# protolambda/go-kzg

Measured on AMD Instinct MI355X. Metric: KZG commitments/sec (CommitToPoly, 4096-element blob); FK20 half: value_fk20_4096, higher is better.
Workload: dtype u32; 1 GPU; CommitToPoly, 4096-coeff blobs, eth/trusted_setup.json monomial setup (s=1337), 4096 blobs/step/GPU resident in HBM, fixed-base table budget 110 GB (library default 110 GB: signed 16-bit windows, 8 of them walked by both GLV halves of every scalar, 103 GB; see table_sweep); global_batch=4096, parallelism=dp1 (independent blobs, no data-path collective)

## Files before the change

go-kzg_amd/csrc/capi_fk20.hip:

```cpp
#include "capi_common.hpp"

__global__ void k_fk20_x(const g1j *secret, uint64_t n, uint64_t l, uint64_t k, g1j *x ) {
    uint64_t t = blockIdx.x * (uint64_t)blockDim.x + threadIdx.x;
    if (t >= l * k) return;
    uint64_t off = t / k, i = t % k;
    x[t] = (i + 1 < k) ? secret[n - l - 1 - off - i * l] : g1_inf();
}

static int fk20_core_new(kzg_hip_kzg *ks, uint64_t n2, uint64_t l, fk20_core *c) {
    kzg_hip_fft *fs = ks->fs;
    dev_guard g(fs);
    hipStream_t s = fs->stream;
    uint64_t n = n2 / 2, k = n / l, k2 = 2 * k;
    c->ks = ks; c->n2 = n2; c->l = l; c->k = k;
    dtmp<g1j> d_x(s), d_f(s);
    CHK(d_x.alloc(l * k)); CHK(d_f.alloc(l * k2));
    HIPCHK(hipMalloc((void **)&c->d_files, l * k2 * sizeof(g1j)));
    hipLaunchKernelGGL(k_fk20_x, dim3((uint32_t)((l * k + 255) / 256)), dim3(256), 0, s, ks->d_secret, n, l, k, d_x.p);
    CHK(g1_fft_rows(fs, s, d_x.p, k, k, d_f.p, k2, l, 0));
    launch_g1_normalize(s, d_f.p, c->d_files, l * k2);
    HIPCHK(hipGetLastError());
    {
        double budget_gb = table_budget_gb("KZG_HIP_FK20_FB_BUDGET_GB", 48.0, 12.0);
        uint64_t npts = l * k2;
        const bool glv = fb_glv_enabled();
        dtmp<g1a> d_fa(s);
        if (npts >= 64) { CHK(d_fa.alloc(npts)); launch_g1_to_affine(s, c->d_files, d_fa.p, npts); }
        for (uint32_t cc = glv ? 16 : 14; cc >= 4 && npts >= 64; cc--) {
            const uint32_t nwin = glv ? fb_windows_glv(cc) : fb_windows(cc);
            if (glv && cc > 4 && fb_windows_glv(cc - 1) == nwin) continue;
            double bytes = (double)nwin * (double)npts * (double)(1u << (cc - 1)) * sizeof(g1a);
            if (bytes > budget_gb * 1e9) continue;
            g1a *tab = nullptr;
            if (hipMalloc((void **)&tab, (size_t)nwin * npts * (1u << (cc - 1)) * sizeof(g1a)) != hipSuccess) { (void)hipGetLastError(); continue; }
            hipError_t e = launch_fb_build(s, d_fa.p, npts, cc, nwin, tab);
            if (e == hipSuccess) e = hipStreamSynchronize(s);
            if (e != hipSuccess) { (void)hipGetLastError(); hipFree(tab); continue; }
            c->d_files_fb = tab; c->fb_c = cc; c->fb_nwin = nwin; c->fb_glv = glv;
            break;
        }
    }
    HIPCHK(hipStreamSynchronize(s));
    return KZG_HIP_OK;
}

int fk20_hext(fk20_core *c, hipStream_t s, const fr *d_poly, uint64_t poly_stride, uint64_t n, uint64_t batch, uint64_t j0, uint64_t cnt, g1j *d_hext) {
    kzg_hip_fft *fs = c->ks->fs;
    uint64_t l = c->l, k2 = 2 * c->k;
    dtmp<fr> d_tc(s), d_cf(s);
    CHK(d_tc.alloc(batch * l * k2)); CHK(d_cf.alloc(batch * l * k2));
    launch_toeplitz_coeffs(s, d_poly, poly_stride, n, l, batch, d_tc.p, fs->d_inv_pow2 + ilog2(k2));
    fr_fft_rows(fs, s, d_tc.p, k2, k2, d_cf.p, k2, batch * l, 0);
    if (c->d_files_fb) {
        if (l == 1) launch_fb_mul_vec(s, c->d_files_fb, l * k2, c->fb_c, c->fb_nwin, d_cf.p, k2, j0, cnt, batch, d_hext, c->fb_glv);
        else if (batch * cnt >= device_simd_lanes()) launch_fb_mul_vec_files(s, c->d_files_fb, l * k2, c->fb_c, c->fb_nwin, d_cf.p, k2, j0, cnt, batch, d_hext, c->fb_glv);
        else {
            dtmp<g1j> d_tmp(s);
            CHK(d_tmp.alloc(batch * l * cnt));
            launch_fb_mul_vec(s, c->d_files_fb, l * k2, c->fb_c, c->fb_nwin, d_cf.p, k2, j0, cnt, batch, d_tmp.p, c->fb_glv);
            launch_g1_sum_files(s, d_tmp.p, l, cnt, batch, d_hext);
        }
// ... 13 lines not shown
    HIPCHK(hipGetLastError());
    return KZG_HIP_OK;
}
int fk20_finish(fk20_core *c, hipStream_t s, const g1j *d_hext, uint64_t batch, int da, int bit_reverse, g1j *d_out) {
    kzg_hip_fft *fs = c->ks->fs;
    const uint64_t k2 = 2 * c->k;
    dtmp<g1j> d_a(s);
    CHK(d_a.alloc(batch * k2));
    CHK(g1_fft_rows(fs, s, d_hext, k2, k2, d_a.p, k2, batch, 1, nullptr, c->k));
    return fk20_finish_from_h(c, s, d_a.p, batch, da, bit_reverse, d_out);
}
static bool fk20_pass1_fused_ok(const fk20_core *c, uint64_t batch) {
    static const bool off = [] { const char *e = getenv("KZG_HIP_FK20_PASS1"); return e && e[0] == '0'; }();
    const uint64_t k2 = 2 * c->k;
    return !off && c->l == 1 && c->d_files_fb && k2 >= 32 && g1_fft_direct_mode(k2, batch) && g1_fft_direct_logr(k2, batch) == 4;
}
static int fk20_run_pass1_fused(fk20_core *c, hipStream_t s, const fr *d_poly, uint64_t poly_stride, uint64_t n, uint64_t batch, int da, int bit_reverse, g1j *d_out) {
    kzg_hip_fft *fs = c->ks->fs;
    const uint64_t k2 = 2 * c->k;
    dtmp<fr> d_tc(s), d_cf(s); dtmp<g1j> d_p1(s), d_a(s), d_tmp(s);
    CHK(d_tc.alloc(batch * k2)); CHK(d_cf.alloc(batch * k2)); CHK(d_p1.alloc(batch * k2)); CHK(d_a.alloc(batch * k2)); CHK(d_tmp.alloc(batch * k2));
    launch_toeplitz_coeffs(s, d_poly, poly_stride, n, 1, batch, d_tc.p, fs->d_inv_pow2 + ilog2(k2));
    fr_fft_rows(fs, s, d_tc.p, k2, k2, d_cf.p, k2, batch, 0);
    launch_fb_direct_pass1(s, c->d_files_fb, k2, c->fb_c, c->fb_nwin, d_cf.p, fs->d_reversed, fs->W, batch, 4, d_p1.p, c->fb_glv);
    launch_g1_fft_direct(s, d_p1.p, k2, k2, d_a.p, d_tmp.p, k2, batch, fs->d_reversed, fs->W, nullptr, 4, g1_fft_direct_lanes(k2, batch), 4, c->k);
    HIPCHK(hipGetLastError());
    return fk20_finish_from_h(c, s, d_a.p, batch, da, bit_reverse, d_out);
}
static bool fk20_fused_ok(const fk20_core *c, uint64_t batch, int da) {
    static const bool off = [] { const char *e = getenv("KZG_HIP_FK20_FUSE"); return e && e[0] == '0'; }();
    const uint64_t k2 = 2 * c->k;
    return !off && c->l == 1 && c->d_files_fb && k2 >= 8 && !g1_fft_direct_mode(k2, batch) && (da || !g1_fft_direct_mode(c->k, batch));
}
static int fk20_run_fused(fk20_core *c, hipStream_t s, const fr *d_poly, uint64_t poly_stride, uint64_t n, uint64_t batch, int da, int bit_reverse, g1j *d_out) {
    kzg_hip_fft *fs = c->ks->fs;
    const uint64_t k2 = 2 * c->k;
    dtmp<fr> d_tc(s), d_cf(s); dtmp<g1j> d_a(s), d_b(s);
    CHK(d_tc.alloc(batch * k2)); CHK(d_cf.alloc(batch * k2)); CHK(d_a.alloc(batch * k2)); CHK(d_b.alloc(batch * k2));
    launch_toeplitz_coeffs(s, d_poly, poly_stride, n, 1, batch, d_tc.p, fs->d_inv_pow2 + ilog2(k2));
    fr_fft_rows(fs, s, d_tc.p, k2, k2, d_cf.p, k2, batch, 0);
    launch_fb_mul_vec_dif2(s, c->d_files_fb, k2, c->fb_c, c->fb_nwin, d_cf.p, fs->d_reversed, fs->W, batch, d_a.p, c->fb_glv);
    for (uint64_t m = k2 / 8; m >= 1; m >>= 1) launch_g1_fft_stage_dif(s, d_a.p, k2, batch, m, fs->d_glv_reversed, fs->d_wnaf_reversed, fs->W);
    if (!da) {
        const uint64_t k = c->k;
        launch_g1_take_even(s, d_a.p, d_b.p, batch * k);
        for (uint64_t m = 1; m < k; m <<= 1) launch_g1_fft_stage(s, d_b.p, k, batch, m, fs->d_glv_expanded, fs->d_wnaf_expanded, fs->W);
        if (bit_reverse) { launch_g1_bitrev_copy(s, d_b.p, k, k, d_a.p, k, batch); launch_g1_normalize(s, d_a.p, d_out, batch * k, true); }
        else launch_g1_normalize(s, d_b.p, d_out, batch * k, true);
        HIPCHK(hipGetLastError());
        return KZG_HIP_OK;
    }
    launch_g1_clear_odd(s, d_a.p, batch * k2);
    for (uint64_t m = 1; m < k2; m <<= 1) launch_g1_fft_stage(s, d_a.p, k2, batch, m, fs->d_glv_expanded, fs->d_wnaf_expanded, fs->W);
    if (bit_reverse) { launch_g1_bitrev_copy(s, d_a.p, k2, k2, d_b.p, k2, batch); launch_g1_normalize(s, d_b.p, d_out, batch * k2, true); }
    else launch_g1_normalize(s, d_a.p, d_out, batch * k2, true);
    HIPCHK(hipGetLastError());
    return KZG_HIP_OK;
}
static uint64_t fk20_padded_batch(uint64_t batch) {
    static const bool off = [] { const char *e = getenv("KZG_HIP_FK20_PAD"); return e && e[0] == '0'; }();
    if (off) return batch;
    if (batch > 16 && batch < 32) return 32;
    if (batch > 32 && (batch & 7)) {
        const uint64_t p = (batch + 7) & ~7ull;
        if ((p - batch) * 32 <= batch) return p;
    }
    return batch;
// ... 222 lines not shown
```

go-kzg_amd/csrc/g1_coop_kernels.hpp:

```cpp
#pragma once
#include "internal.hpp"
#include "g1_quad.hpp"
#include <stdlib.h>
#include <string.h>

namespace kzg {

#ifndef G1_BLOCK
#define G1_BLOCK 256
#endif
struct g1jq_slot { uint32_t w[39]; uint32_t inf; uint32_t pad; };
#define G1_DIRECT_BLOCK 64
static inline uint32_t ilog2_coop(uint64_t v) { uint32_t r = 0; while ((1ull << r) < v) r++; return r; }

template <bool DIF, bool WNAF, int L> __global__ __launch_bounds__(G1_BLOCK, 2) void k_g1_fft_stage_quad(g1j *data, uint32_t logn, uint64_t m, const fr *roots, const int8_t *wnaf, uint64_t W, uint64_t total, uint64_t batch) {
    const uint64_t t4 = blockIdx.x * (uint64_t)blockDim.x + threadIdx.x;
    const uint32_t role = (uint32_t)(t4 & (uint64_t)(L - 1));
    const uint64_t t = t4 / L;
    if (t >= total) return;
    const uint64_t half = 1ull << (logn - 1), groups = half / m;
    const uint64_t j = t / (groups * batch), rem = t % (groups * batch), b = rem / groups, g = rem % groups;
    g1j *row = data + (b << logn);
    const uint64_t i0 = g * 2 * m + j, i1 = i0 + m;
    g1j y = row[i1];
// ... 49 lines not shown
            g1jq dq;
            const int st = QMUL(g1jq_unpack(d_), dq);
            d_ = st == 1 ? g1jq_pack(dq) : st == 2 ? packed : g1_inf();
        }
        if (role == 0) { row[i0] = s_; row[i1] = d_; }
    }
}
#undef QMUL
static inline bool g1_quad_wnaf(uint64_t n, uint64_t batch, uint64_t m, int lanes) {
    static const bool off = [] { const char *e = getenv("KZG_HIP_G1_MUL"); return e && e[0] == 'r'; }();
    return !off && ((n / 2 / m) * batch * lanes) % 64 == 0;
}
template <bool DIF> static inline void launch_stage_coop(hipStream_t s, int lanes, g1j *data, uint64_t n, uint64_t batch, uint64_t m, const fr *roots, const int8_t *wnaf, uint64_t W,
                                                  uint64_t total) {
    static const bool once = [] {
        hipFuncSetAttribute(reinterpret_cast<const void *>(&k_g1_fft_stage_quad<DIF, true, 4>), hipFuncAttributeMaxDynamicSharedMemorySize, 96 * 1024);
        hipFuncSetAttribute(reinterpret_cast<const void *>(&k_g1_fft_stage_quad<DIF, false, 4>), hipFuncAttributeMaxDynamicSharedMemorySize, 96 * 1024);
        hipFuncSetAttribute(reinterpret_cast<const void *>(&k_g1_fft_stage_quad<DIF, true, 2>), hipFuncAttributeMaxDynamicSharedMemorySize, 96 * 1024);
        hipFuncSetAttribute(reinterpret_cast<const void *>(&k_g1_fft_stage_quad<DIF, false, 2>), hipFuncAttributeMaxDynamicSharedMemorySize, 96 * 1024);
        return true; }();
    (void)once;
    const size_t lds = total * lanes <= device_simd_lanes() ? 96 * 1024 : 0;
    const dim3 qg((uint32_t)((lanes * total + G1_BLOCK - 1) / G1_BLOCK));
    const uint32_t logn = ilog2_coop(n);
    const bool wn = g1_quad_wnaf(n, batch, m, lanes);
    if (lanes == 4) {
        if (wn) hipLaunchKernelGGL((k_g1_fft_stage_quad<DIF, true, 4>), qg, dim3(G1_BLOCK), lds, s, data, logn, m, roots, wnaf, W, total, batch);
        else hipLaunchKernelGGL((k_g1_fft_stage_quad<DIF, false, 4>), qg, dim3(G1_BLOCK), lds, s, data, logn, m, roots, wnaf, W, total, batch);
    } else {
        if (wn) hipLaunchKernelGGL((k_g1_fft_stage_quad<DIF, true, 2>), qg, dim3(G1_BLOCK), lds, s, data, logn, m, roots, wnaf, W, total, batch);
        else hipLaunchKernelGGL((k_g1_fft_stage_quad<DIF, false, 2>), qg, dim3(G1_BLOCK), lds, s, data, logn, m, roots, wnaf, W, total, batch);
    }
}
template <int L> __global__ __launch_bounds__(G1_DIRECT_BLOCK, 2) void k_g1_fft_direct_coop(const g1j *in, uint64_t in_stride, uint64_t n_valid, g1j *out, uint32_t logn,
                                                                                          uint32_t logR, uint64_t Ns, const fr *roots, uint64_t W, const fr *scale, uint64_t total,
                                                                                          uint32_t logT, uint32_t logU) {
    __shared__ g1jq_slot buf[G1_DIRECT_BLOCK / L];
    const uint32_t tid = threadIdx.x, role = tid & (uint32_t)(L - 1), item = tid / L;
    const uint64_t t = (blockIdx.x * (uint64_t)blockDim.x + tid) / L;
    const uint64_t n = 1ull << logn, R = 1ull << logR, cols = n >> logR, T = 1ull << logT;
    const uint32_t tt = (uint32_t)(t & (T - 1));
    const uint64_t u = (t >> logT) & ((1ull << logU) - 1), jb = t >> (logT + logU), j = jb % cols, b = jb / cols;
    const bool live = t < total;
    g1jq_acc acc; acc.inf = true;
    uint64_t oidx = 0;
    if (live) {
        const uint64_t k = j & (Ns - 1), idx = j + (uint64_t)tt * cols;
        oidx = b * n + (j - k) * R + k + u * Ns;
        g1j x = idx < n_valid ? in[b * in_stride + idx] : g1_inf();
        if (!is_inf(x)) {
            const uint64_t e = ((uint64_t)tt * (cols / Ns) * (Ns * u + k)) & (n - 1);
            if (e == 0 && !scale) { acc.v = g1jq_unpack(x); acc.inf = false; }
            else {
                fr sc = roots[e * (W >> logn)];
                if (scale) sc = mul(sc, *scale);
                g1aq tbl[8]; fq dz[7]; g1j packed;
                const int st = g1_mul_glv_regular_quad<L>(g1jq_unpack(x), glv_split_signed(from_mont<FrP>(sc)), tbl, dz, acc.v, packed, role);
                if (st == 2) { acc.inf = is_inf(packed); if (!acc.inf) acc.v = g1jq_unpack(packed); } else acc.inf = st == 0;
            }
        }
    }
#define COOP_STORE(i) do { _Pragma("unroll") for (int q = 0; q < 13; q++) { buf[i].w[q] = acc.v.x.l[q]; buf[i].w[13 + q] = acc.v.y.l[q]; buf[i].w[26 + q] = acc.v.z.l[q]; } \
                           buf[i].inf = acc.inf ? 1u : 0u; } while (0)
    if (role == 0) COOP_STORE(item);
    __syncthreads();
#pragma nounroll
// ... 16 lines not shown
```

go-kzg_amd/csrc/internal.hpp:

```cpp
#pragma once
#include <hip/hip_runtime.h>
#include <stdint.h>
#include "field.hpp"
#include "g1.hpp"

namespace kzg {

void launch_fr_fft(hipStream_t s, const fr *in, uint64_t in_stride, uint64_t n_in, fr *out, uint64_t n, uint64_t batch,
                   const fr *roots, uint64_t W, const fr *scale, const uint32_t *tw4096 = nullptr, const fr *roots_l = nullptr);
void launch_das_ext(hipStream_t s, fr *vals, uint64_t n, uint64_t batch, const fr *expanded, const fr *reversed, uint64_t W,
                    const fr *inv_n, const uint32_t *tw2048 = nullptr);
void launch_toeplitz_coeffs(hipStream_t s, const fr *poly, uint64_t poly_stride, uint64_t n, uint64_t l, uint64_t batch, fr *out,
                            const fr *scale);
void launch_quotient_linear(hipStream_t s, const fr *poly, uint64_t poly_stride, uint64_t n, uint64_t batch, const fr *x, fr *q, uint64_t q_stride);
void launch_fr_from_u64(hipStream_t s, const uint64_t *in, uint64_t in_stride, fr *out, uint64_t n);
void launch_fr_zero_tails(hipStream_t s, fr *rows, uint64_t n_max, uint64_t batch, const uint64_t *lens, uint64_t lens_stride);
void launch_fr_any_nonzero(hipStream_t s, const fr *vals, uint64_t n, uint32_t *flag);
void launch_fr_powers(hipStream_t s, const fr *base, uint64_t n, fr *out);

void launch_fr_from_le32(hipStream_t s, const uint8_t *in, fr *out, uint64_t per_blob, uint64_t batch, uint32_t *bad);
void launch_fr_to_le32(hipStream_t s, const fr *in, uint8_t *out, uint64_t n);
void launch_fr_bitrev_gather(hipStream_t s, const fr *in, fr *out, uint64_t n);
constexpr uint64_t ZERO_TREE_LEAF = 16;
void launch_zero_leaves(hipStream_t s, const fr *expanded, uint64_t stride, const uint64_t *missing, uint64_t n_missing, uint64_t leaves, fr *a);
void launch_zero_pair_products(hipStream_t s, const fr *f, uint64_t m, uint64_t pairs, fr *out);
void launch_zero_join(hipStream_t s, fr *c, const fr *a, uint64_t d, uint64_t pairs);
void launch_zero_unpad(hipStream_t s, const fr *root, uint64_t pad, uint64_t n_missing, uint64_t length, fr *poly);
void launch_fr_mul_table_rows(hipStream_t s, fr *data, const fr *table, uint64_t stride, uint64_t n, uint64_t batch);
void launch_poly_lincomb(hipStream_t s, const fr *vectors, uint64_t stride, const fr *scalars, uint64_t count, uint64_t n, fr *out);
void launch_eth_quotient(hipStream_t s, const fr *poly, uint64_t poly_stride, const fr *domain, uint64_t n, uint64_t batch, const fr *z, uint64_t z_stride,
                         const fr *inv_n, fr *q, fr *y_out, uint32_t *flag, uint64_t dom_stride = 1, fr *scratch = nullptr);
uint64_t eth_quotient_scratch_elems(uint64_t n, uint64_t batch);

void launch_fr_scale_by_inv_powers(hipStream_t s, fr *c, const fr *x, uint64_t n, fr *xpow_n);

void launch_zero_eval_direct(hipStream_t s, const fr *expanded, uint64_t stride, const uint64_t *missing, uint64_t n_missing, uint64_t length, fr *zero_eval);
void launch_fr_scale_by_powers(hipStream_t s, fr *poly, const fr *base, uint64_t n);
void launch_fr_pointwise(hipStream_t s, const fr *a, const fr *b, const uint8_t *present, fr *out, uint64_t n, int mode, uint32_t *flag);

void launch_g1_mul_vec(hipStream_t s, const g1j *pts, uint64_t pts_mod, const fr *scalars, uint64_t s_stride, uint64_t n, g1j *out);
hipError_t launch_g1_file_msm(hipStream_t s, const g1j *files, const fr *scalars, uint64_t nfiles, uint64_t k2, uint64_t j0, uint64_t cnt,
                              uint64_t batch, g1j *out);
void launch_g1_bitrev_copy(hipStream_t s, const g1j *in, uint64_t in_stride, uint64_t n_valid, g1j *out, uint64_t n, uint64_t batch);
void launch_g1_fft_stage(hipStream_t s, g1j *data, uint64_t n, uint64_t batch, uint64_t m, const fr *roots, const int8_t *wnaf, uint64_t W);
void launch_g1_fft_stage_dif(hipStream_t s, g1j *data, uint64_t n, uint64_t batch, uint64_t m, const fr *roots, const int8_t *wnaf, uint64_t W);
void launch_g1_clear_odd(hipStream_t s, g1j *data, uint64_t n_total);
void launch_g1_take_even(hipStream_t s, const g1j *in, g1j *out, uint64_t total);
bool g1_quad_enabled();
void launch_fb_direct_pass1(hipStream_t s, const g1a *table, uint64_t table_n, uint32_t c, uint32_t nwin, const fr *scalars, const fr *roots, uint64_t W, uint64_t batch,
                            uint32_t logR, g1j *out, bool glv = false);
void launch_g1_stage_coop_dif(hipStream_t s, int lanes, g1j *data, uint64_t n, uint64_t batch, uint64_t m, const fr *roots, const int8_t *wnaf, uint64_t W, uint64_t total);
void launch_g1_stage_coop_dit(hipStream_t s, int lanes, g1j *data, uint64_t n, uint64_t batch, uint64_t m, const fr *roots, const int8_t *wnaf, uint64_t W, uint64_t total);
void launch_g1_direct_coop(hipStream_t s, int lanes, uint32_t wgs, size_t pad_lds, const g1j *src, uint64_t src_stride, uint64_t src_valid, g1j *dst, uint32_t logn, uint32_t logR,
                           uint64_t Ns, const fr *roots, uint64_t W, const fr *sc, uint64_t total, uint32_t logT, uint32_t logU);
void launch_g1_fft_direct(hipStream_t s, const g1j *in, uint64_t in_stride, uint64_t n_valid, g1j *data, g1j *tmp, uint64_t n, uint64_t batch, const fr *roots,
                          uint64_t W, const fr *scale, uint32_t max_logr = 4, int lanes = 1, uint32_t bits_done = 0, uint64_t n_out = 0);
void launch_g1_normalize(hipStream_t s, const g1j *in, g1j *out, uint64_t n, bool to_kilic = false);
void launch_fr_inv_test(hipStream_t s, const fr *in, uint64_t n, fr *out_coop, fr *out_lane, fr *out_block);
void launch_fp_inv_both(hipStream_t s, const fp *in, fp *out_coop, fp *out_lane, uint64_t n, int mode);
void launch_g1_from_kilic(hipStream_t s, g1j *data, uint64_t n);
void launch_g1_to_affine(hipStream_t s, const g1j *in, g1a *out, uint64_t n);
void launch_g1_compress(hipStream_t s, const g1j *in, uint8_t *out48, uint64_t n);
void launch_g1_decompress(hipStream_t s, const uint8_t *in48, g1j *out, uint64_t n, uint32_t *bad_flag);
void launch_g1_fixed_base_powers(hipStream_t s, const fr *powers, uint64_t n, g1j *out);

uint64_t device_simd_lanes();
inline uint64_t device_simds() { return device_simd_lanes() / 64; }
struct msm_plan {
    uint32_t c;
    uint32_t nwin;
    uint32_t nb;
    uint32_t ngroups;
    uint32_t fixed;
    uint32_t glv;
    uint64_t table_n;
};
inline bool msm_index_range_ok(const msm_plan &p, uint64_t n) { return n < (1ull << 27) && 2 * p.table_n < (1ull << 30); }
size_t msm_workspace_bytes(const msm_plan &p, uint64_t n, uint64_t batch);
void launch_msm(hipStream_t s, const msm_plan &p, const g1a *table, const fr *scalars, uint64_t sc_stride, uint64_t n, uint64_t batch, void *workspace, g1j *out,
                bool to_kilic);
void launch_msm_window_table(hipStream_t s, const g1a *pts, uint64_t n, uint32_t c, uint32_t nwin, g1j *tmp, g1a *out);

size_t fb_partials_bytes(uint64_t n, uint64_t batch);
hipError_t launch_fb_build(hipStream_t s, const g1a *pts, uint64_t n, uint32_t c, uint32_t nwin, g1a *table);
void launch_fb_msm(hipStream_t s, const g1a *table, uint64_t table_n, uint32_t c, uint32_t nwin, const fr *scalars, uint64_t sc_stride, uint64_t n,
                   uint64_t batch, void *partials, g1j *out, bool to_kilic, bool glv = false, bool projective = false);

void launch_fb_mul_vec(hipStream_t s, const g1a *table, uint64_t table_n, uint32_t c, uint32_t nwin, const fr *scalars, uint64_t row, uint64_t j0,
                       uint64_t cnt, uint64_t batch, g1j *out, bool glv = false);
void launch_fb_mul_vec_dif2(hipStream_t s, const g1a *table, uint64_t table_n, uint32_t c, uint32_t nwin, const fr *scalars, const fr *roots, uint64_t W,
                            uint64_t batch, g1j *out, bool glv = false);
void launch_fb_mul_vec_files(hipStream_t s, const g1a *table, uint64_t table_n, uint32_t c, uint32_t nwin, const fr *scalars, uint64_t row, uint64_t j0,
                             uint64_t cnt, uint64_t batch, g1j *out, bool glv = false);
void launch_g1_sum_files(hipStream_t s, const g1j *tmp, uint64_t nfiles, uint64_t cnt, uint64_t batch, g1j *out);

struct g2j; struct g2_prepared;
void launch_g2_from_compressed(hipStream_t s, const uint8_t *in96, g2j *out_kilic, uint64_t n, uint32_t *bad_flag);
void launch_g2_prepare(hipStream_t s, const g2j *in_kilic, uint64_t n, g2_prepared *out);
void launch_pairs_g1_from_kilic(hipStream_t s, const g1j *a1, const g1j *b1, uint64_t n, g1j *p0, g1j *p1);
void launch_kzg_check_inputs(hipStream_t s, const g1j *c, const g1j *pi, const fr *ys, const g1j *es, const fr *bs, uint64_t n, g1j *p0, g1j *p1);
void launch_fr_rows_scale_by_inv_powers(hipStream_t s, fr *c, uint64_t np, const fr *xs, uint64_t count, fr *xpow_n);
void launch_eth_check_inputs(hipStream_t s, const uint8_t *c48, const uint8_t *zs, const uint8_t *ys, const uint8_t *pi48, uint64_t n, g1j *p0, g1j *p1, uint8_t *status);
void launch_pairing_check(hipStream_t s, bool shared_lines, const g2_prepared *q0, const g2_prepared *q1, const g1j *p0, const g1j *p1, uint64_t n, uint8_t *ok);
void launch_pairing_value(hipStream_t s, const g1j *g1_kilic, const g2_prepared *q, uint64_t n, fp *out);

void prof_begin(hipStream_t s, const char *name);
void prof_end(hipStream_t s, const char *name);

}
```

go-kzg_amd/csrc/k_g1.hip:

```cpp
#define KZG_MULQ_NOINLINE 1
#include "internal.hpp"
#include "coop_inv.hpp"
#include <stdlib.h>

namespace kzg {

#ifndef G1_BLOCK
#define G1_BLOCK 256
#endif

__device__ __forceinline__ uint32_t bitrev32g(uint32_t v, uint32_t bits) { return bits ? (__brev(v) >> (32 - bits)) : 0; }

__device__ __forceinline__ g1j g1_mul_fr(const g1j &p, const fr &k_mont) {
    if (is_inf(p)) return g1_inf();
    g1aq tbl[8]; fq dz[7]; g1jq q; g1j packed;
    const int st = g1_mul_glv_regular_aq<false>(g1jq_unpack(p), glv_split_signed(from_mont<FrP>(k_mont)), tbl, dz, q, packed);
    return st == 1 ? g1jq_pack(q) : st == 2 ? packed : g1_inf();
}

__global__ __launch_bounds__(G1_BLOCK, 2) void k_g1_mul_vec(const g1j *pts, uint64_t pts_mod, const fr *scalars, uint64_t s_stride, uint64_t n,
                                                         g1j *out) {
    uint64_t t = blockIdx.x * (uint64_t)blockDim.x + threadIdx.x;
    if (t >= n) return;
    g1j p = pts[t % pts_mod];
// ... 155 lines not shown
    }
    row[i0] = s_; row[i1] = d_;
}
void launch_g1_fft_stage_dif(hipStream_t s, g1j *data, uint64_t n, uint64_t batch, uint64_t m, const fr *roots, const int8_t *wnaf, uint64_t W) {
    uint64_t total = n / 2 * batch;
    if (!total) return;
    prof_begin(s, "g1_fft_stage");
    if (const int lanes = g1_stage_lanes(total); lanes > 1) {
        launch_g1_stage_coop_dif(s, lanes, data, n, batch, m, roots, wnaf, W, total);
        prof_end(s, "g1_fft_stage");
        return;
    }
    const dim3 grid((uint32_t)((total + G1_BLOCK - 1) / G1_BLOCK)), block(G1_BLOCK);
    if (g1_wnaf_rows_pay(n, batch, m)) hipLaunchKernelGGL(k_g1_fft_stage_dif<true>, grid, block, 0, s, data, ilog2g(n), m, roots, wnaf, W, total, batch);
    else hipLaunchKernelGGL(k_g1_fft_stage_dif<false>, grid, block, 0, s, data, ilog2g(n), m, roots, wnaf, W, total, batch);
    prof_end(s, "g1_fft_stage");
}
__global__ void k_g1_clear_odd(g1j *data, uint64_t total_pairs) {
    uint64_t t = blockIdx.x * (uint64_t)blockDim.x + threadIdx.x;
    if (t < total_pairs) data[2 * t + 1] = g1_inf();
}
void launch_g1_clear_odd(hipStream_t s, g1j *data, uint64_t n_total) {
    if (n_total < 2) return;
    hipLaunchKernelGGL(k_g1_clear_odd, dim3((uint32_t)((n_total / 2 + 255) / 256)), dim3(256), 0, s, data, n_total / 2);
}
__global__ void k_g1_take_even(const g1j *in, g1j *out, uint64_t total) {
    uint64_t t = blockIdx.x * (uint64_t)blockDim.x + threadIdx.x;
    if (t < total) out[t] = in[2 * t];
}
void launch_g1_take_even(hipStream_t s, const g1j *in, g1j *out, uint64_t total) {
    if (!total) return;
    hipLaunchKernelGGL(k_g1_take_even, dim3((uint32_t)((total + 255) / 256)), dim3(256), 0, s, in, out, total);
}
void launch_g1_fft_stage(hipStream_t s, g1j *data, uint64_t n, uint64_t batch, uint64_t m, const fr *roots, const int8_t *wnaf, uint64_t W) {
    uint64_t total = n / 2 * batch;
    if (!total) return;
    prof_begin(s, "g1_fft_stage");
    static const int forced = [] { const char *e = getenv("KZG_HIP_G1_MUL"); return !e ? -1 : e[0] == 'r' ? 0 : e[0] == 'w' ? 4 : -1; }();
    const uint64_t per_twiddle = (n / 2 / m) * batch;
    const int mode = forced >= 0 ? forced : ((per_twiddle % 64 == 0 || per_twiddle >= 256) ? 4 : 0);
    if (const int lanes = g1_stage_lanes(total); lanes > 1) {
        launch_g1_stage_coop_dit(s, lanes, data, n, batch, m, roots, wnaf, W, total);
        prof_end(s, "g1_fft_stage");
        return;
    }
    const dim3 grid((uint32_t)((total + G1_BLOCK - 1) / G1_BLOCK)), block(G1_BLOCK);
    const uint32_t logn = ilog2g(n);
    switch (mode) {
    case 4:
        if (g1_wnaf_rows_pay(n, batch, m)) hipLaunchKernelGGL((k_g1_fft_stage<4, true>), grid, block, 0, s, data, logn, m, roots, wnaf, W, total, batch);
        else hipLaunchKernelGGL((k_g1_fft_stage<4, false>), grid, block, 0, s, data, logn, m, roots, wnaf, W, total, batch);
        break;
    default: hipLaunchKernelGGL(k_g1_fft_stage<0>, grid, block, 0, s, data, logn, m, roots, wnaf, W, total, batch); break;
    }
    prof_end(s, "g1_fft_stage");
}

struct g1jq_slot { uint32_t w[39]; uint32_t inf; uint32_t pad; };
#define G1_DIRECT_BLOCK 64
__global__ __launch_bounds__(G1_DIRECT_BLOCK, 2) void k_g1_fft_direct(const g1j *in, uint64_t in_stride, uint64_t n_valid, g1j *out, uint32_t logn, uint32_t logR,
                                                            uint64_t Ns, const fr *roots, uint64_t W, const fr *scale, uint64_t total, uint32_t logT, uint32_t logU) {
    __shared__ g1jq_slot buf[G1_DIRECT_BLOCK];
    const uint32_t tid = threadIdx.x;
    const uint64_t t = blockIdx.x * (uint64_t)blockDim.x + tid;
    const uint64_t n = 1ull << logn, R = 1ull << logR, cols = n >> logR, T = 1ull << logT;
    const uint32_t tt = (uint32_t)(t & (T - 1));
    const uint64_t u = (t >> logT) & ((1ull << logU) - 1), jb = t >> (logT + logU), j = jb % cols, b = jb / cols;
    const bool live = t < total;
    g1jq_acc acc; acc.inf = true;
    uint64_t oidx = 0;
    if (live) {
        const uint64_t k = j & (Ns - 1), idx = j + (uint64_t)tt * cols;
        oidx = b * n + (j - k) * R + k + u * Ns;
        g1j x = idx < n_valid ? in[b * in_stride + idx] : g1_inf();
        if (!is_inf(x)) {
            const uint64_t e = ((uint64_t)tt * (cols / Ns) * (Ns * u + k)) & (n - 1);
            if (e == 0 && !scale) { acc.v = g1jq_unpack(x); acc.inf = false; }
            else {
                fr sc = roots[e * (W >> logn)];
                if (scale) sc = mul(sc, *scale);
                g1aq tbl[8]; fq dz[7]; g1j packed;
                const int st = g1_mul_glv_regular_aq<true>(g1jq_unpack(x), glv_split_signed(from_mont<FrP>(sc)), tbl, dz, acc.v, packed);
                if (st == 2) { acc.inf = is_inf(packed); if (!acc.inf) acc.v = g1jq_unpack(packed); } else acc.inf = st == 0;
            }
        }
    }
    auto store = [&](uint32_t i) {
#pragma unroll
// ... 205 lines not shown
```

go-kzg_amd/csrc/k_msm.hip:

```cpp
#include "internal.hpp"
#include "g1_quad.hpp"
#include "coop_inv.hpp"
#include <atomic>
#include <cstring>

namespace kzg {

#define MSM_SORT_T 1024
#define MSM_ACC_BLOCK 128
#define MSM_NB 128

struct fb_partial { uint32_t w[52]; uint32_t inf; };
__device__ __forceinline__ void fb_partial_store(fb_partial &o, const g1x_acc &a) {
#pragma unroll
    for (int i = 0; i < 13; i++) { o.w[i] = a.v.x.l[i]; o.w[13 + i] = a.v.y.l[i]; o.w[26 + i] = a.v.zz.l[i]; o.w[39 + i] = a.v.zzz.l[i]; }
    o.inf = a.inf ? 1u : 0u;
}
__device__ __forceinline__ void fb_partial_load(const fb_partial &p, g1xq &v) {
#pragma unroll
    for (int i = 0; i < 13; i++) { v.x.l[i] = p.w[i]; v.y.l[i] = p.w[13 + i]; v.zz.l[i] = p.w[26 + i]; v.zzz.l[i] = p.w[39 + i]; }
}

template <uint32_t DELTA> __device__ __forceinline__ uint32_t lane_down(uint32_t v) {
    if constexpr (DELTA < 16) return (uint32_t)__builtin_amdgcn_update_dpp((int)v, (int)v, 0x100 + DELTA, 0xf, 0xf, false);
// ... 726 lines not shown
        if (!xa.inf) { acc.v = g1jq_unpack(xa.to_jac()); acc.inf = false; }
    }
#define FBP_STORE(i_) do { _Pragma("unroll") for (int q_ = 0; q_ < 13; q_++) { buf[i_].w[q_] = acc.v.x.l[q_]; buf[i_].w[13 + q_] = acc.v.y.l[q_]; buf[i_].w[26 + q_] = acc.v.z.l[q_]; } \
                           buf[i_].inf = acc.inf ? 1u : 0u; } while (0)
    FBP_STORE(tid);
    __syncthreads();
#pragma nounroll
    for (uint32_t off = (uint32_t)R / 2; off >= 1; off >>= 1) {
        if (tt < off && !buf[tid + off].inf) {
            g1jq q;
#pragma unroll
            for (int i = 0; i < 13; i++) { q.x.l[i] = buf[tid + off].w[i]; q.y.l[i] = buf[tid + off].w[13 + i]; q.z.l[i] = buf[tid + off].w[26 + i]; }
            acc.add(q);
            FBP_STORE(tid);
        }
        __syncthreads();
    }
#undef FBP_STORE
    if (live && tt == 0) out[b * n + j * R + u] = acc.inf ? g1_inf() : g1jq_pack(acc.v);
}
void launch_fb_direct_pass1(hipStream_t s, const g1a *table, uint64_t table_n, uint32_t c, uint32_t nwin, const fr *scalars, const fr *roots, uint64_t W, uint64_t batch,
                            uint32_t logR, g1j *out, bool glv) {
    uint32_t logn = 0;
    while ((1ull << logn) < table_n) logn++;
    const uint64_t total = (batch * table_n) << logR, wgs = (total + 63) / 64;
    prof_begin(s, "fb_mul_vec");
    if (glv) hipLaunchKernelGGL(k_fb_direct_pass1<true>, dim3((uint32_t)wgs), dim3(64), wgs <= device_simds() ? 24 * 1024 : 0, s, table, table_n, c, nwin, 1u << (c - 1), scalars, roots, W, logn, logR,
                                total, out);
    else hipLaunchKernelGGL(k_fb_direct_pass1<false>, dim3((uint32_t)wgs), dim3(64), wgs <= device_simds() ? 24 * 1024 : 0, s, table, table_n, c, nwin, 1u << (c - 1), scalars, roots, W, logn, logR,
                            total, out);
    prof_end(s, "fb_mul_vec");
}

template <bool GLV> __global__ __launch_bounds__(FB_BLOCK, 2) void k_fb_mul_vec_dif2(const g1a *table, uint64_t table_n, uint32_t c, uint32_t nwin, uint32_t D, const fr *scalars,
                                                              const fr *roots, uint64_t W, uint64_t total, g1j *out) {
    uint64_t t = blockIdx.x * (uint64_t)blockDim.x + threadIdx.x;
    if (t >= total) return;
    const uint64_t N = table_n, q = N >> 2;
    const uint64_t i = t % q, o = (t / q) & 3u, b = t / N;
    const uint64_t rs = W / N;
    g1x_acc acc; acc.init();
#pragma nounroll
    for (uint32_t pass = GLV ? 0u : 1u; pass < 2; pass++) {
#pragma nounroll
        for (uint32_t term = 0; term < 4; term++) {
            const uint64_t pi = i + term * q;
            uint64_t e; uint32_t sg;
            if (o == 0) { e = 0; sg = 0; }
            else if (o == 1) { e = 2 * i; sg = term & 1u; }
            else if (o == 2) { e = i + ((term & 1u) ? q : 0); sg = term >> 1; }
            else { e = 3 * i + ((term & 1u) ? q : 0); sg = (term == 1 || term == 2) ? 1u : 0u; }
            fr kmont = scalars[b * N + pi];
            if (e) kmont = mul(kmont, roots[(e & (N - 1)) * rs]);
            const fr k = from_mont<FrP>(kmont);
            fb_walk_term<GLV>(acc, table, table_n, c, nwin, D, pi, k, sg, pass == 0);
        }
        if (GLV && pass == 0) acc_apply_phi(acc);
    }
    out[b * N + o * q + i] = acc.to_jac();
}
void launch_fb_mul_vec_dif2(hipStream_t s, const g1a *table, uint64_t table_n, uint32_t c, uint32_t nwin, const fr *scalars, const fr *roots, uint64_t W,
                            uint64_t batch, g1j *out, bool glv) {
    uint64_t total = batch * table_n;
    if (!total) return;
    prof_begin(s, "fb_mul_vec");
    if (glv) hipLaunchKernelGGL(k_fb_mul_vec_dif2<true>, dim3((uint32_t)((total + FB_BLOCK - 1) / FB_BLOCK)), dim3(FB_BLOCK), 0, s, table, table_n, c, nwin, 1u << (c - 1), scalars,
                                roots, W, total, out);
    else hipLaunchKernelGGL(k_fb_mul_vec_dif2<false>, dim3((uint32_t)((total + FB_BLOCK - 1) / FB_BLOCK)), dim3(FB_BLOCK), 0, s, table, table_n, c, nwin, 1u << (c - 1), scalars,
                            roots, W, total, out);
    prof_end(s, "fb_mul_vec");
}
template <bool GLV> __global__ __launch_bounds__(FB_BLOCK, 2) void k_fb_mul_vec_files(const g1a *table, uint64_t table_n, uint32_t c, uint32_t nwin, uint32_t D, const fr *scalars,
                                                               uint64_t i0, uint64_t cnt, uint64_t row, uint64_t total, g1j *out) {
    uint64_t t = blockIdx.x * (uint64_t)blockDim.x + threadIdx.x;
    if (t >= total) return;
    const uint64_t jj = t % cnt, b = t / cnt, nfiles = table_n / row;
    g1x_acc acc; acc.init();
#pragma nounroll
    for (uint32_t pass = GLV ? 0u : 1u; pass < 2; pass++) {
#pragma nounroll
        for (uint64_t f = 0; f < nfiles; f++) {
            const uint64_t i = f * row + i0 + jj;
            const fr k = from_mont<FrP>(scalars[b * table_n + i]);
            fb_walk_term<GLV>(acc, table, table_n, c, nwin, D, i, k, 0u, pass == 0);
        }
        if (GLV && pass == 0) acc_apply_phi(acc);
    }
    out[t] = acc.to_jac();
}
void launch_fb_mul_vec_files(hipStream_t s, const g1a *table, uint64_t table_n, uint32_t c, uint32_t nwin, const fr *scalars, uint64_t row, uint64_t j0,
                             uint64_t cnt, uint64_t batch, g1j *out, bool glv) {
    uint64_t total = batch * cnt;
    if (!total) return;
    prof_begin(s, "fb_mul_vec");
    if (glv) hipLaunchKernelGGL(k_fb_mul_vec_files<true>, dim3((uint32_t)((total + FB_BLOCK - 1) / FB_BLOCK)), dim3(FB_BLOCK), 0, s, table, table_n, c, nwin, 1u << (c - 1), scalars,
                                j0, cnt, row, total, out);
    else hipLaunchKernelGGL(k_fb_mul_vec_files<false>, dim3((uint32_t)((total + FB_BLOCK - 1) / FB_BLOCK)), dim3(FB_BLOCK), 0, s, table, table_n, c, nwin, 1u << (c - 1), scalars,
                            j0, cnt, row, total, out);
    prof_end(s, "fb_mul_vec");
}
void launch_fb_mul_vec(hipStream_t s, const g1a *table, uint64_t table_n, uint32_t c, uint32_t nwin, const fr *scalars, uint64_t row, uint64_t j0,
                       uint64_t cnt, uint64_t batch, g1j *out, bool glv) {
// ... 107 lines not shown
```

Measured before the change: 104,000 commitments/s.

## Add half-size FK20 path computing only even outputs via odd/even split

When only the non-extended proofs are needed (da=0), a new path computes the k even outputs of the 2k-point G1 FFT directly. It splits the work into an odd-index half-size fixed-base DIF product followed by a half-size DIF, a twist and a DIT, plus an even-index strided term scaled by k, and adds the two results. This removes the full 2k-length G1 FFT stages and the take-even step, at the cost of an extra twist kernel of scalar multiplications and a second fixed-base pass. A tunable minimum point count for building the fixed-base table is also added.

```diff
diff --git a/go-kzg_amd/csrc/capi_fk20.hip b/go-kzg_amd/csrc/capi_fk20.hip
--- a/go-kzg_amd/csrc/capi_fk20.hip
+++ b/go-kzg_amd/csrc/capi_fk20.hip
@@ -24,9 +24,10 @@
         double budget_gb = table_budget_gb("KZG_HIP_FK20_FB_BUDGET_GB", 48.0, 12.0);
         uint64_t npts = l * k2;
         const bool glv = fb_glv_enabled();
+        static const uint64_t min_pts = [] { const char *e = getenv("KZG_HIP_FK20_FB_MIN_POINTS"); const uint64_t v = e ? strtoull(e, nullptr, 10) : 0; return v ? v : 64ull; }();
         dtmp<g1a> d_fa(s);
-        if (npts >= 64) { CHK(d_fa.alloc(npts)); launch_g1_to_affine(s, c->d_files, d_fa.p, npts); }
-        for (uint32_t cc = glv ? 16 : 14; cc >= 4 && npts >= 64; cc--) {
+        if (npts >= min_pts) { CHK(d_fa.alloc(npts)); launch_g1_to_affine(s, c->d_files, d_fa.p, npts); }
+        for (uint32_t cc = glv ? 16 : 14; cc >= 4 && npts >= min_pts; cc--) {
             const uint32_t nwin = glv ? fb_windows_glv(cc) : fb_windows(cc);
             if (glv && cc > 4 && fb_windows_glv(cc - 1) == nwin) continue;
             double bytes = (double)nwin * (double)npts * (double)(1u << (cc - 1)) * sizeof(g1a);
@@ -106,7 +107,30 @@
     const uint64_t k2 = 2 * c->k;
     return !off && c->l == 1 && c->d_files_fb && k2 >= 8 && !g1_fft_direct_mode(k2, batch) && (da || !g1_fft_direct_mode(c->k, batch));
 }
+static bool fk20_half_ok() {
+    static const bool off = [] { const char *e = getenv("KZG_HIP_FK20_HALF"); return e && e[0] == '0'; }();
+    return !off;
+}
+static int fk20_run_fused_half(fk20_core *c, hipStream_t s, const fr *d_poly, uint64_t poly_stride, uint64_t n, uint64_t batch, int bit_reverse, g1j *d_out) {
+    kzg_hip_fft *fs = c->ks->fs;
+    const uint64_t k = c->k, k2 = 2 * k;
+    dtmp<fr> d_tc(s), d_cf(s); dtmp<g1j> d_u(s), d_e(s);
+    CHK(d_tc.alloc(batch * k2)); CHK(d_cf.alloc(batch * k2)); CHK(d_u.alloc(batch * k)); CHK(d_e.alloc(batch * k));
+    launch_toeplitz_coeffs(s, d_poly, poly_stride, n, 1, batch, d_tc.p, fs->d_inv_pow2 + ilog2(k2));
+    fr_fft_rows(fs, s, d_tc.p, k2, k2, d_cf.p, k2, batch, 0);
+    launch_fb_mul_vec_dif2(s, c->d_files_fb, k2, c->fb_c, c->fb_nwin, d_cf.p, fs->d_reversed, fs->W, batch, d_u.p, c->fb_glv, true);
+    launch_fb_mul_vec_strided(s, c->d_files_fb, k2, c->fb_c, c->fb_nwin, d_cf.p, 0, 2, k, batch, fr_from_u64(k), d_e.p, c->fb_glv);
+    for (uint64_t m = k / 8; m >= 1; m >>= 1) launch_g1_fft_stage_dif(s, d_u.p, k, batch, m, fs->d_glv_reversed, fs->d_wnaf_reversed, fs->W);
+    launch_g1_twist(s, d_u.p, k, batch, fs->d_glv_reversed, fs->d_wnaf_reversed, fs->W);
+    for (uint64_t m = 1; m < k; m <<= 1) launch_g1_fft_stage(s, d_u.p, k, batch, m, fs->d_glv_expanded, fs->d_wnaf_expanded, fs->W);
+    launch_g1_add_vec(s, d_u.p, d_e.p, d_u.p, batch * k);
+    if (bit_reverse) { launch_g1_bitrev_copy(s, d_u.p, k, k, d_e.p, k, batch); launch_g1_normalize(s, d_e.p, d_out, batch * k, true); }
+    else launch_g1_normalize(s, d_u.p, d_out, batch * k, true);
+    HIPCHK(hipGetLastError());
+    return KZG_HIP_OK;
+}
 static int fk20_run_fused(fk20_core *c, hipStream_t s, const fr *d_poly, uint64_t poly_stride, uint64_t n, uint64_t batch, int da, int bit_reverse, g1j *d_out) {
+    if (!da && fk20_half_ok()) return fk20_run_fused_half(c, s, d_poly, poly_stride, n, batch, bit_reverse, d_out);
     kzg_hip_fft *fs = c->ks->fs;
     const uint64_t k2 = 2 * c->k;
     dtmp<fr> d_tc(s), d_cf(s); dtmp<g1j> d_a(s), d_b(s);
diff --git a/go-kzg_amd/csrc/g1_coop_kernels.hpp b/go-kzg_amd/csrc/g1_coop_kernels.hpp
--- a/go-kzg_amd/csrc/g1_coop_kernels.hpp
+++ b/go-kzg_amd/csrc/g1_coop_kernels.hpp
@@ -105,6 +105,28 @@
         else hipLaunchKernelGGL((k_g1_fft_stage_quad<DIF, false, 2>), qg, dim3(G1_BLOCK), lds, s, data, logn, m, roots, wnaf, W, total, batch);
     }
 }
+template <bool WNAF, int L> __global__ __launch_bounds__(G1_BLOCK, 2) void k_g1_twist_quad(g1j *data, uint32_t logn, const fr *roots, const int8_t *wnaf, uint64_t stride, uint64_t total, uint64_t batch) {
+    const uint64_t t4 = blockIdx.x * (uint64_t)blockDim.x + threadIdx.x;
+    const uint32_t role = (uint32_t)(t4 & (uint64_t)(L - 1));
+    const uint64_t t = t4 / L;
+    if (t >= total) return;
+    const uint64_t p = t / batch, b = t % batch;
+    const uint64_t j = logn ? (__brev((uint32_t)p) >> (32 - logn)) : 0;
+    if (!j) return;
+    g1j *ptr = data + (b << logn) + p;
+    const g1j y = *ptr;
+    if (is_inf(y)) return;
+    const uint64_t ti = j * stride;
+    const fr kk = roots[ti];
+    glv_halves h;
+#pragma unroll
+    for (int i = 0; i < 4; i++) { h.k1[i] = kk.l[i]; h.k2[i] = kk.l[4 + i]; }
+    h.neg1 = h.neg2 = 0;
+    g1aq tbl[8]; fq dz[7]; g1j packed; g1jq q;
+    const int st = WNAF ? g1_mul_glv_wnaf_quad<L>(g1jq_unpack(y), kk, tbl, dz, wnaf + ti * KZG_WNAF_ROW, q, packed, role)
+                        : g1_mul_glv_regular_quad<L>(g1jq_unpack(y), h, tbl, dz, q, packed, role);
+    if (role == 0) *ptr = st == 1 ? g1jq_pack(q) : st == 2 ? packed : g1_inf();
+}
 template <int L> __global__ __launch_bounds__(G1_DIRECT_BLOCK, 2) void k_g1_fft_direct_coop(const g1j *in, uint64_t in_stride, uint64_t n_valid, g1j *out, uint32_t logn,
                                                                                           uint32_t logR, uint64_t Ns, const fr *roots, uint64_t W, const fr *scale, uint64_t total,
                                                                                           uint32_t logT, uint32_t logU) {
diff --git a/go-kzg_amd/csrc/internal.hpp b/go-kzg_amd/csrc/internal.hpp
--- a/go-kzg_amd/csrc/internal.hpp
+++ b/go-kzg_amd/csrc/internal.hpp
@@ -46,11 +46,14 @@
 void launch_g1_fft_stage_dif(hipStream_t s, g1j *data, uint64_t n, uint64_t batch, uint64_t m, const fr *roots, const int8_t *wnaf, uint64_t W);
 void launch_g1_clear_odd(hipStream_t s, g1j *data, uint64_t n_total);
 void launch_g1_take_even(hipStream_t s, const g1j *in, g1j *out, uint64_t total);
+void launch_g1_twist(hipStream_t s, g1j *data, uint64_t n, uint64_t batch, const fr *roots, const int8_t *wnaf, uint64_t W);
+void launch_g1_add_vec(hipStream_t s, const g1j *a, const g1j *b, g1j *out, uint64_t total);
 bool g1_quad_enabled();
 void launch_fb_direct_pass1(hipStream_t s, const g1a *table, uint64_t table_n, uint32_t c, uint32_t nwin, const fr *scalars, const fr *roots, uint64_t W, uint64_t batch,
                             uint32_t logR, g1j *out, bool glv = false);
 void launch_g1_stage_coop_dif(hipStream_t s, int lanes, g1j *data, uint64_t n, uint64_t batch, uint64_t m, const fr *roots, const int8_t *wnaf, uint64_t W, uint64_t total);
 void launch_g1_stage_coop_dit(hipStream_t s, int lanes, g1j *data, uint64_t n, uint64_t batch, uint64_t m, const fr *roots, const int8_t *wnaf, uint64_t W, uint64_t total);
+void launch_g1_twist_coop(hipStream_t s, int lanes, g1j *data, uint64_t n, uint64_t batch, const fr *roots, const int8_t *wnaf, uint64_t W, uint64_t total);
 void launch_g1_direct_coop(hipStream_t s, int lanes, uint32_t wgs, size_t pad_lds, const g1j *src, uint64_t src_stride, uint64_t src_valid, g1j *dst, uint32_t logn, uint32_t logR,
                            uint64_t Ns, const fr *roots, uint64_t W, const fr *sc, uint64_t total, uint32_t logT, uint32_t logU);
 void launch_g1_fft_direct(hipStream_t s, const g1j *in, uint64_t in_stride, uint64_t n_valid, g1j *data, g1j *tmp, uint64_t n, uint64_t batch, const fr *roots,
@@ -89,7 +92,9 @@
 void launch_fb_mul_vec(hipStream_t s, const g1a *table, uint64_t table_n, uint32_t c, uint32_t nwin, const fr *scalars, uint64_t row, uint64_t j0,
                        uint64_t cnt, uint64_t batch, g1j *out, bool glv = false);
 void launch_fb_mul_vec_dif2(hipStream_t s, const g1a *table, uint64_t table_n, uint32_t c, uint32_t nwin, const fr *scalars, const fr *roots, uint64_t W,
-                            uint64_t batch, g1j *out, bool glv = false);
+                            uint64_t batch, g1j *out, bool glv = false, bool odd = false);
+void launch_fb_mul_vec_strided(hipStream_t s, const g1a *table, uint64_t table_n, uint32_t c, uint32_t nwin, const fr *scalars, uint64_t i0, uint64_t step, uint64_t cnt,
+                               uint64_t batch, const fr &scale, g1j *out, bool glv = false);
 void launch_fb_mul_vec_files(hipStream_t s, const g1a *table, uint64_t table_n, uint32_t c, uint32_t nwin, const fr *scalars, uint64_t row, uint64_t j0,
                              uint64_t cnt, uint64_t batch, g1j *out, bool glv = false);
 void launch_g1_sum_files(hipStream_t s, const g1j *tmp, uint64_t nfiles, uint64_t cnt, uint64_t batch, g1j *out);
diff --git a/go-kzg_amd/csrc/k_g1.hip b/go-kzg_amd/csrc/k_g1.hip
--- a/go-kzg_amd/csrc/k_g1.hip
+++ b/go-kzg_amd/csrc/k_g1.hip
@@ -211,13 +211,16 @@
     if (!total) return;
     hipLaunchKernelGGL(k_g1_take_even, dim3((uint32_t)((total + 255) / 256)), dim3(256), 0, s, in, out, total);
 }
+static int g1_stage_mode(uint64_t per_twiddle) {
+    static const int forced = [] { const char *e = getenv("KZG_HIP_G1_MUL"); return !e ? -1 : e[0] == 'r' ? 0 : e[0] == 'w' ? 4 : -1; }();
+    return forced >= 0 ? forced : ((per_twiddle % 64 == 0 || per_twiddle >= 256) ? 4 : 0);
+}
 void launch_g1_fft_stage(hipStream_t s, g1j *data, uint64_t n, uint64_t batch, uint64_t m, const fr *roots, const int8_t *wnaf, uint64_t W) {
     uint64_t total = n / 2 * batch;
     if (!total) return;
     prof_begin(s, "g1_fft_stage");
-    static const int forced = [] { const char *e = getenv("KZG_HIP_G1_MUL"); return !e ? -1 : e[0] == 'r' ? 0 : e[0] == 'w' ? 4 : -1; }();
     const uint64_t per_twiddle = (n / 2 / m) * batch;
-    const int mode = forced >= 0 ? forced : ((per_twiddle % 64 == 0 || per_twiddle >= 256) ? 4 : 0);
+    const int mode = g1_stage_mode(per_twiddle);
     if (const int lanes = g1_stage_lanes(total); lanes > 1) {
         launch_g1_stage_coop_dit(s, lanes, data, n, batch, m, roots, wnaf, W, total);
         prof_end(s, "g1_fft_stage");
@@ -233,6 +236,58 @@
     default: hipLaunchKernelGGL(k_g1_fft_stage<0>, grid, block, 0, s, data, logn, m, roots, wnaf, W, total, batch); break;
     }
     prof_end(s, "g1_fft_stage");
+}
+
+template <int MODE, bool PRE = false> __global__ __launch_bounds__(G1_BLOCK, 2) void k_g1_twist(g1j *data, uint32_t logn, const fr *roots, const int8_t *wnaf, uint64_t stride, uint64_t total, uint64_t batch) {
+    uint64_t t = blockIdx.x * (uint64_t)blockDim.x + threadIdx.x;
+    if (t >= total) return;
+    const uint64_t p = t / batch, b = t % batch;
+    const uint64_t j = bitrev32g((uint32_t)p, logn);
+    if (!j) return;
+    g1j *ptr = data + (b << logn) + p;
+    const g1j y = *ptr;
+    if (is_inf(y)) return;
+    const uint64_t ti = j * stride;
+    g1aq tbl[8]; fq dz[7]; g1jq q; g1j packed;
+    int st;
+    if (MODE == 4) {
+        if (PRE) st = g1_mul_glv_wnaf_aq_pre_q<true, true>(g1jq_unpack(y), roots[ti], tbl, dz, wnaf + ti * KZG_WNAF_ROW, q, packed);
+        else { int8_t dg1[132], dg2[132]; st = g1_mul_glv_wnaf_aq<true, true>(y, roots[ti], tbl, dz, dg1, dg2, 1, q, packed); }
+    } else {
+        const fr kk = roots[ti];
+        glv_halves h;
+#pragma unroll
+        for (int i = 0; i < 4; i++) { h.k1[i] = kk.l[i]; h.k2[i] = kk.l[4 + i]; }
+        h.neg1 = h.neg2 = 0;
+        st = g1_mul_glv_regular_aq<true>(g1jq_unpack(y), h, tbl, dz, q, packed);
+    }
+    *ptr = st == 1 ? g1jq_pack(q) : st == 2 ? packed : g1_inf();
+}
+void launch_g1_twist(hipStream_t s, g1j *data, uint64_t n, uint64_t batch, const fr *roots, const int8_t *wnaf, uint64_t W) {
+    uint64_t total = n * batch;
+    if (!total || n < 2) return;
+    prof_begin(s, "g1_twist");
+    if (const int lanes = g1_stage_lanes(total); lanes > 1) {
+        launch_g1_twist_coop(s, lanes, data, n, batch, roots, wnaf, W, total);
+        prof_end(s, "g1_twist");
+        return;
+    }
+    const dim3 grid((uint32_t)((total + G1_BLOCK - 1) / G1_BLOCK)), block(G1_BLOCK);
+    const uint32_t logn = ilog2g(n);
+    const uint64_t stride = W / (2 * n);
+    if (g1_stage_mode(batch) == 4) {
+        if (batch >= (uint64_t)KZG_WNAF_ROWS_MIN) hipLaunchKernelGGL((k_g1_twist<4, true>), grid, block, 0, s, data, logn, roots, wnaf, stride, total, batch);
+        else hipLaunchKernelGGL((k_g1_twist<4, false>), grid, block, 0, s, data, logn, roots, wnaf, stride, total, batch);
+    } else hipLaunchKernelGGL(k_g1_twist<0>, grid, block, 0, s, data, logn, roots, wnaf, stride, total, batch);
+    prof_end(s, "g1_twist");
+}
+__global__ __launch_bounds__(G1_BLOCK, 2) void k_g1_add_vec(const g1j *a, const g1j *b, g1j *out, uint64_t total) {
+    uint64_t t = blockIdx.x * (uint64_t)blockDim.x + threadIdx.x;
+    if (t < total) out[t] = g1_add(a[t], b[t]);
+}
+void launch_g1_add_vec(hipStream_t s, const g1j *a, const g1j *b, g1j *out, uint64_t total) {
+    if (!total) return;
+    hipLaunchKernelGGL(k_g1_add_vec, dim3((uint32_t)((total + G1_BLOCK - 1) / G1_BLOCK)), dim3(G1_BLOCK), 0, s, a, b, out, total);
 }
 
 struct g1jq_slot { uint32_t w[39]; uint32_t inf; uint32_t pad; };
diff --git a/go-kzg_amd/csrc/k_g1_coop_twist.hip b/go-kzg_amd/csrc/k_g1_coop_twist.hip
--- /dev/null
+++ b/go-kzg_amd/csrc/k_g1_coop_twist.hip
@@ -0,0 +1,25 @@
+#define KZG_MULQ_NOINLINE 1
+#include "g1_coop_kernels.hpp"
+namespace kzg {
+void launch_g1_twist_coop(hipStream_t s, int lanes, g1j *data, uint64_t n, uint64_t batch, const fr *roots, const int8_t *wnaf, uint64_t W, uint64_t total) {
+    static const bool once = [] {
+        hipFuncSetAttribute(reinterpret_cast<const void *>(&k_g1_twist_quad<true, 4>), hipFuncAttributeMaxDynamicSharedMemorySize, 96 * 1024);
+        hipFuncSetAttribute(reinterpret_cast<const void *>(&k_g1_twist_quad<false, 4>), hipFuncAttributeMaxDynamicSharedMemorySize, 96 * 1024);
+        hipFuncSetAttribute(reinterpret_cast<const void *>(&k_g1_twist_quad<true, 2>), hipFuncAttributeMaxDynamicSharedMemorySize, 96 * 1024);
+        hipFuncSetAttribute(reinterpret_cast<const void *>(&k_g1_twist_quad<false, 2>), hipFuncAttributeMaxDynamicSharedMemorySize, 96 * 1024);
+        return true; }();
+    (void)once;
+    const size_t lds = total * lanes <= device_simd_lanes() ? 96 * 1024 : 0;
+    const dim3 qg((uint32_t)((lanes * total + G1_BLOCK - 1) / G1_BLOCK));
+    const uint32_t logn = ilog2_coop(n);
+    const uint64_t stride = W / (2 * n);
+    const bool wn = g1_quad_wnaf(n, batch, n / 2, lanes);
+    if (lanes == 4) {
+        if (wn) hipLaunchKernelGGL((k_g1_twist_quad<true, 4>), qg, dim3(G1_BLOCK), lds, s, data, logn, roots, wnaf, stride, total, batch);
+        else hipLaunchKernelGGL((k_g1_twist_quad<false, 4>), qg, dim3(G1_BLOCK), lds, s, data, logn, roots, wnaf, stride, total, batch);
+    } else {
+        if (wn) hipLaunchKernelGGL((k_g1_twist_quad<true, 2>), qg, dim3(G1_BLOCK), lds, s, data, logn, roots, wnaf, stride, total, batch);
+        else hipLaunchKernelGGL((k_g1_twist_quad<false, 2>), qg, dim3(G1_BLOCK), lds, s, data, logn, roots, wnaf, stride, total, batch);
+    }
+}
+}
diff --git a/go-kzg_amd/csrc/k_msm.hip b/go-kzg_amd/csrc/k_msm.hip
--- a/go-kzg_amd/csrc/k_msm.hip
+++ b/go-kzg_amd/csrc/k_msm.hip
@@ -782,11 +782,11 @@
     prof_end(s, "fb_mul_vec");
 }
 
-template <bool GLV> __global__ __launch_bounds__(FB_BLOCK, 2) void k_fb_mul_vec_dif2(const g1a *table, uint64_t table_n, uint32_t c, uint32_t nwin, uint32_t D, const fr *scalars,
+template <bool GLV, bool ODD = false> __global__ __launch_bounds__(FB_BLOCK, 2) void k_fb_mul_vec_dif2(const g1a *table, uint64_t table_n, uint32_t c, uint32_t nwin, uint32_t D, const fr *scalars,
                                                               const fr *roots, uint64_t W, uint64_t total, g1j *out) {
     uint64_t t = blockIdx.x * (uint64_t)blockDim.x + threadIdx.x;
     if (t >= total) return;
-    const uint64_t N = table_n, q = N >> 2;
+    const uint64_t N = ODD ? table_n >> 1 : table_n, q = N >> 2;
     const uint64_t i = t % q, o = (t / q) & 3u, b = t / N;
     const uint64_t rs = W / N;
     g1x_acc acc; acc.init();
@@ -794,13 +794,13 @@
     for (uint32_t pass = GLV ? 0u : 1u; pass < 2; pass++) {
 #pragma nounroll
         for (uint32_t term = 0; term < 4; term++) {
-            const uint64_t pi = i + term * q;
+            const uint64_t pi = ODD ? 2 * (i + term * q) + 1 : i + term * q;
             uint64_t e; uint32_t sg;
             if (o == 0) { e = 0; sg = 0; }
             else if (o == 1) { e = 2 * i; sg = term & 1u; }
             else if (o == 2) { e = i + ((term & 1u) ? q : 0); sg = term >> 1; }
             else { e = 3 * i + ((term & 1u) ? q : 0); sg = (term == 1 || term == 2) ? 1u : 0u; }
-            fr kmont = scalars[b * N + pi];
+            fr kmont = scalars[b * table_n + pi];
             if (e) kmont = mul(kmont, roots[(e & (N - 1)) * rs]);
             const fr k = from_mont<FrP>(kmont);
             fb_walk_term<GLV>(acc, table, table_n, c, nwin, D, pi, k, sg, pass == 0);
@@ -810,14 +810,38 @@
     out[b * N + o * q + i] = acc.to_jac();
 }
 void launch_fb_mul_vec_dif2(hipStream_t s, const g1a *table, uint64_t table_n, uint32_t c, uint32_t nwin, const fr *scalars, const fr *roots, uint64_t W,
-                            uint64_t batch, g1j *out, bool glv) {
-    uint64_t total = batch * table_n;
+                            uint64_t batch, g1j *out, bool glv, bool odd) {
+    uint64_t total = batch * (odd ? table_n / 2 : table_n);
     if (!total) return;
+    const dim3 grid((uint32_t)((total + FB_BLOCK - 1) / FB_BLOCK)), block(FB_BLOCK);
+    const uint32_t D = 1u << (c - 1);
     prof_begin(s, "fb_mul_vec");
-    if (glv) hipLaunchKernelGGL(k_fb_mul_vec_dif2<true>, dim3((uint32_t)((total + FB_BLOCK - 1) / FB_BLOCK)), dim3(FB_BLOCK), 0, s, table, table_n, c, nwin, 1u << (c - 1), scalars,
-                                roots, W, total, out);
-    else hipLaunchKernelGGL(k_fb_mul_vec_dif2<false>, dim3((uint32_t)((total + FB_BLOCK - 1) / FB_BLOCK)), dim3(FB_BLOCK), 0, s, table, table_n, c, nwin, 1u << (c - 1), scalars,
-                            roots, W, total, out);
+    if (odd) {
+        if (glv) hipLaunchKernelGGL((k_fb_mul_vec_dif2<true, true>), grid, block, 0, s, table, table_n, c, nwin, D, scalars, roots, W, total, out);
+        else hipLaunchKernelGGL((k_fb_mul_vec_dif2<false, true>), grid, block, 0, s, table, table_n, c, nwin, D, scalars, roots, W, total, out);
+    } else if (glv) hipLaunchKernelGGL((k_fb_mul_vec_dif2<true>), grid, block, 0, s, table, table_n, c, nwin, D, scalars, roots, W, total, out);
+    else hipLaunchKernelGGL((k_fb_mul_vec_dif2<false>), grid, block, 0, s, table, table_n, c, nwin, D, scalars, roots, W, total, out);
+    prof_end(s, "fb_mul_vec");
+}
+template <bool GLV> __global__ __launch_bounds__(FB_BLOCK, 2) void k_fb_mul_vec_strided(const g1a *table, uint64_t table_n, uint32_t c, uint32_t nwin, uint32_t D, const fr *scalars,
+                                                                 uint64_t i0, uint64_t step, uint64_t cnt, fr scale, uint64_t total, g1j *out) {
+    uint64_t t = blockIdx.x * (uint64_t)blockDim.x + threadIdx.x;
+    if (t >= total) return;
+    const uint64_t jj = t % cnt, b = t / cnt, i = i0 + jj * step;
+    const fr k = from_mont<FrP>(mul(scalars[b * table_n + i], scale));
+    g1x_acc acc; acc.init();
+    if (GLV) { fb_walk_term<true>(acc, table, table_n, c, nwin, D, i, k, 0u, true); acc_apply_phi(acc); }
+    fb_walk_term<GLV>(acc, table, table_n, c, nwin, D, i, k, 0u, false);
+    out[t] = acc.to_jac();
+}
+void launch_fb_mul_vec_strided(hipStream_t s, const g1a *table, uint64_t table_n, uint32_t c, uint32_t nwin, const fr *scalars, uint64_t i0, uint64_t step, uint64_t cnt,
+                               uint64_t batch, const fr &scale, g1j *out, bool glv) {
+    uint64_t total = batch * cnt;
+    if (!total) return;
+    const dim3 grid((uint32_t)((total + FB_BLOCK - 1) / FB_BLOCK)), block(FB_BLOCK);
+    prof_begin(s, "fb_mul_vec");
+    if (glv) hipLaunchKernelGGL(k_fb_mul_vec_strided<true>, grid, block, 0, s, table, table_n, c, nwin, 1u << (c - 1), scalars, i0, step, cnt, scale, total, out);
+    else hipLaunchKernelGGL(k_fb_mul_vec_strided<false>, grid, block, 0, s, table, table_n, c, nwin, 1u << (c - 1), scalars, i0, step, cnt, scale, total, out);
     prof_end(s, "fb_mul_vec");
 }
 template <bool GLV> __global__ __launch_bounds__(FB_BLOCK, 2) void k_fb_mul_vec_files(const g1a *table, uint64_t table_n, uint32_t c, uint32_t nwin, uint32_t D, const fr *scalars,
```

Measured after the change: 104,200 commitments/s (median of 6 runs). No clear change (+0.2%).
